# nomic-ai/contrastors

Measured on AMD Instinct MI355X. Metric: query-doc pairs/sec (whole node), nomic-bert-2048 seq128 global-batch 16384, higher is better.
Workload: dtype bf16

## Files before the change

contrastors_amd/csrc/gemm_bf16_v7.hip:

```cpp
#include "cx_common.h"
#include "../../include/contrastors_hip.h"
#include "gemm_params.h"
#include <type_traits>

namespace {

#ifndef CX_V7_NT
#define CX_V7_NT 3
#endif

template <int IMM>
__device__ __forceinline__ void v7_dma_m0(uint32_t base) {
    asm volatile("s_add_u32 m0, %0, %1" ::"s"(base), "n"(IMM) : "memory", "scc");
}
__device__ __forceinline__ void v7_dma_ld(uint32_t off, const bf16_t* base) {
    asm volatile("global_load_lds_dwordx4 %0, %1" ::"v"(off), "s"(base) : "memory");
}
template <int IMM>
__device__ __forceinline__ void v7_dma_full(uint32_t slot_base, uint32_t off, const bf16_t* base) {
    asm volatile("s_add_u32 m0, %0, %1\n\ts_nop 0\n\tglobal_load_lds_dwordx4 %2, %3" ::"s"(slot_base), "n"(IMM), "v"(off), "s"(base)
                 : "memory", "scc");
}
typedef unsigned int v4u7 __attribute__((ext_vector_type(4)));
__device__ __forceinline__ __amdgpu_buffer_rsrc_t rsrc7(const void* base, uint32_t bytes) {
// ... 16 lines not shown
}
template <uint32_t IMM>
__device__ __forceinline__ uint32_t vxor7(uint32_t a) {
    uint32_t r;
    asm volatile("v_xor_b32 %0, %2, %1" : "=v"(r) : "v"(a), "i"(IMM));
    return r;
}

typedef __attribute__((address_space(3))) void* lds_void_ptr7;

constexpr int BM7 = 256, BN7 = 128, BK7 = 64;
constexpr int XW7 = 8192;
constexpr int W0_OFF7 = 32768, SP_OFF7 = 49152, W1_OFF7 = 65536;
constexpr int LDS7 = 81920;

#define V7_MFMA(i, w, x) asm volatile("v_mfma_f32_32x32x16_bf16 %0, %1, %2, %0" : "+a"(acc[(i)]) : "v"(w), "v"(x))
#define V7_MFMA_Z(i, w, x) asm volatile("v_mfma_f32_32x32x16_bf16 %0, %1, %2, 0" : "=a"(acc[(i)]) : "v"(w), "v"(x))

struct XFrags7 {
    bf16x8_t f[2][4];
};
struct WFrags7 {
    bf16x8_t f[4];
};

template <int EPI, int DBG = 0>
__global__ __launch_bounds__(256, 2) __attribute__((amdgpu_waves_per_eu(2, 2))) void gemm_bf16_v7_kernel(GemmParams p) {
    extern __shared__ __attribute__((aligned(16))) char dsm[];
    constexpr bool IS_BWD = EPI == GEMM_EPI_SWIGLU_BWD_AG;
    constexpr bool IS_SWIGLU = EPI == GEMM_EPI_SWIGLU_G;
    static_assert(EPI == GEMM_EPI_NONE || IS_BWD || IS_SWIGLU, "v7 serves the plain / residual, SwiGLU (gate save) and SwiGLU-backward (act, gate) forms");
    const int tid = threadIdx.x;
    const int lane = tid & 63;
    const int wave = __builtin_amdgcn_readfirstlane(tid >> 6);
#ifndef CX_PRODUCT
    long long t_begin = 0;
    if (p.trace) t_begin = (long long)__builtin_amdgcn_s_memtime();
#endif
    const int hi_m = lane >> 5, l31_m = lane & 31;
    const int nk = p.K / BK7;
    const int per_xcd = gridDim.x >> 3;
    const int xcd = blockIdx.x & 7, idx = blockIdx.x >> 3;
    const int gn = p.sup_n > 0 ? p.sup_n : 1, gm = 8 / gn;
    const int xi = xcd / gn, xj = xcd - xi * gn;
    const int m_lo = p.tiles_m * xi / gm, m_hi = p.tiles_m * (xi + 1) / gm;
    const int n_lo = p.tiles_n * xj / gn, n_wd = p.tiles_n * (xj + 1) / gn - n_lo;
    const int nloc = (m_hi - m_lo) * n_wd;
    auto tile_of = [&](int round) {
        const int l = round * per_xcd + idx;
        if (l >= nloc) return -1;
        const int q = l / n_wd;
        return ((m_lo + q) << 8) | (n_lo + (l - q * n_wd));
    };

// ... 72 lines not shown
        for (int i = 0; i < slot * p.sup_m; i += 1024) __builtin_amdgcn_s_sleep(16);
    }
    x_setup(cp_tile);
    w_setup(cp_tile);
    v7_dma_full<0>(x_m0, xoff[0], xbase); v7_dma_full<1024>(x_m0, xoff[1], xbase); v7_dma_full<2048>(x_m0, xoff[2], xbase);
    v7_dma_full<3072>(x_m0, xoff[3], xbase); v7_dma_full<4096>(x_m0, xoff[4], xbase); v7_dma_full<5120>(x_m0, xoff[5], xbase);
    v7_dma_full<6144>(x_m0, xoff[6], xbase); v7_dma_full<7168>(x_m0, xoff[7], xbase);
    x_advance();
    v7_dma_full<0>(w_m0, woff[0], wbase); v7_dma_full<4096>(w_m0, woff[1], wbase); v7_dma_full<8192>(w_m0, woff[2], wbase);
    v7_dma_full<12288>(w_m0, woff[3], wbase);
    w_advance();

    const char* xs = dsm + wave * XW7;
    XFrags7 XF;
    WFrags7 W0, W1;
    f32x16_t acc[8];
    auto read_w = [&](WFrags7& f, const char* ws, int ks, int a) {
        if constexpr ((DBG & 4) != 0) return;
        f.f[a] = lds_read_frag(ws, tile64_off(a * 32 + l31_m, ks * 2 + hi_m));
    };
    auto read_x = [&](int b, int ks) {
        if constexpr ((DBG & 32) != 0) return;
        XF.f[b][ks] = lds_read_frag(xs, tile64_off(b * 32 + l31_m, ks * 2 + hi_m));
    };
    if constexpr ((DBG & (4 | 32 | 8)) != 0) {
#pragma unroll
        for (int a = 0; a < 4; ++a) { W0.f[a] = bf16x8_t{}; W1.f[a] = bf16x8_t{}; }
#pragma unroll
        for (int b = 0; b < 2; ++b)
#pragma unroll
            for (int k = 0; k < 4; ++k) XF.f[b][k] = bf16x8_t{};
#pragma unroll
        for (int i = 0; i < 8; ++i) acc[i] = f32x16_t{};
    }
    int ws_slot = 0;
    asm volatile("s_waitcnt vmcnt(0)" ::: "memory");
    __builtin_amdgcn_s_barrier();
#pragma unroll
    for (int a = 0; a < 4; ++a) read_w(W0, dsm + W0_OFF7, 0, a);

#define V7_M0(kind, J)                                                    \
    do {                                                                  \
        if constexpr ((kind) == 1 && (DBG & 1) == 0) v7_dma_m0<(J) * 4096>(w_m0);           \
        if constexpr ((kind) == 2 && (DBG & 1) == 0) v7_dma_m0<(J) * 1024>(x_m0);           \
    } while (0)
#define V7_LD(kind, J)                                                    \
    do {                                                                  \
        if constexpr ((kind) == 1 && (DBG & 1) == 0) v7_dma_ld(woff[(J)], wbase);           \
        if constexpr ((kind) == 2 && (DBG & 1) == 0) v7_dma_ld(xoff[(J)], xbase);           \
    } while (0)
#define V7_SLOT(MMA, i, WC, ks, kind, J, RD)                              \
    do {                                                                  \
        V7_M0(kind, J);                                                   \
        if constexpr ((DBG & 8) == 0) MMA((i), WC.f[(i) & 3], XF.f[(i) >> 2][(ks)]);   \
        V7_LD(kind, J);                                                   \
        RD;                                                               \
        __builtin_amdgcn_sched_barrier(0);                                \
    } while (0)
#define V7_NORD ((void)0)

    auto kt_body = [&](auto first) {
        const char* ws = dsm + (ws_slot ? W1_OFF7 : W0_OFF7);
        const char* nws = dsm + (ws_slot ? W0_OFF7 : W1_OFF7);
        if constexpr ((DBG & 64) == 0) asm volatile("s_waitcnt vmcnt(0)" ::: "memory");
        read_x(0, 0); read_x(1, 0);
        __builtin_amdgcn_sched_barrier(0);
        read_x(0, 1); read_x(1, 1); read_x(0, 2); read_x(1, 2); read_x(0, 3); read_x(1, 3);
        __builtin_amdgcn_sched_barrier(0);
        if constexpr (decltype(first)::value) {
            V7_SLOT(V7_MFMA_Z, 0, W0, 0, 0, 0, read_w(W1, ws, 1, 0));
            V7_SLOT(V7_MFMA_Z, 1, W0, 0, 1, 0, read_w(W1, ws, 1, 1));
            V7_SLOT(V7_MFMA_Z, 2, W0, 0, 1, 1, read_w(W1, ws, 1, 2));
            V7_SLOT(V7_MFMA_Z, 3, W0, 0, 1, 2, read_w(W1, ws, 1, 3));
            V7_SLOT(V7_MFMA_Z, 4, W0, 0, 1, 3, V7_NORD);
            asm volatile("s_waitcnt lgkmcnt(4)" ::: "memory");
            V7_SLOT(V7_MFMA_Z, 5, W0, 0, 2, 0, V7_NORD);
            V7_SLOT(V7_MFMA_Z, 6, W0, 0, 2, 1, V7_NORD);
            V7_SLOT(V7_MFMA_Z, 7, W0, 0, 2, 2, V7_NORD);
        } else {
            V7_SLOT(V7_MFMA, 0, W0, 0, 0, 0, read_w(W1, ws, 1, 0));
            V7_SLOT(V7_MFMA, 1, W0, 0, 1, 0, read_w(W1, ws, 1, 1));
            V7_SLOT(V7_MFMA, 2, W0, 0, 1, 1, read_w(W1, ws, 1, 2));
            V7_SLOT(V7_MFMA, 3, W0, 0, 1, 2, read_w(W1, ws, 1, 3));
            V7_SLOT(V7_MFMA, 4, W0, 0, 1, 3, V7_NORD);
            asm volatile("s_waitcnt lgkmcnt(4)" ::: "memory");
            V7_SLOT(V7_MFMA, 5, W0, 0, 2, 0, V7_NORD);
            V7_SLOT(V7_MFMA, 6, W0, 0, 2, 1, V7_NORD);
            V7_SLOT(V7_MFMA, 7, W0, 0, 2, 2, V7_NORD);
        }
        w_advance();
        V7_SLOT(V7_MFMA, 0, W1, 1, 2, 3, read_w(W0, ws, 2, 0));
        V7_SLOT(V7_MFMA, 1, W1, 1, 2, 4, read_w(W0, ws, 2, 1));
        V7_SLOT(V7_MFMA, 2, W1, 1, 2, 5, read_w(W0, ws, 2, 2));
        V7_SLOT(V7_MFMA, 3, W1, 1, 2, 6, read_w(W0, ws, 2, 3));
        V7_SLOT(V7_MFMA, 4, W1, 1, 2, 7, V7_NORD);
        V7_SLOT(V7_MFMA, 5, W1, 1, 0, 0, V7_NORD);
        V7_SLOT(V7_MFMA, 6, W1, 1, 0, 0, V7_NORD);
        V7_SLOT(V7_MFMA, 7, W1, 1, 0, 0, V7_NORD);
        x_advance();
        V7_SLOT(V7_MFMA, 0, W0, 2, 0, 0, read_w(W1, ws, 3, 0));
        V7_SLOT(V7_MFMA, 1, W0, 2, 0, 0, read_w(W1, ws, 3, 1));
        V7_SLOT(V7_MFMA, 2, W0, 2, 0, 0, read_w(W1, ws, 3, 2));
        V7_SLOT(V7_MFMA, 3, W0, 2, 0, 0, read_w(W1, ws, 3, 3));
        V7_SLOT(V7_MFMA, 4, W0, 2, 0, 0, V7_NORD);
        V7_SLOT(V7_MFMA, 5, W0, 2, 0, 0, V7_NORD);
        V7_SLOT(V7_MFMA, 6, W0, 2, 0, 0, V7_NORD);
        V7_SLOT(V7_MFMA, 7, W0, 2, 0, 0, V7_NORD);
        asm volatile("s_waitcnt lgkmcnt(0)" ::: "memory");
        if constexpr ((DBG & 64) == 0) asm volatile("s_waitcnt vmcnt(8)" ::: "memory");
        if constexpr ((DBG & 2) == 0) __builtin_amdgcn_s_barrier();
        V7_SLOT(V7_MFMA, 0, W1, 3, 0, 0, read_w(W0, nws, 0, 0));
        V7_SLOT(V7_MFMA, 1, W1, 3, 0, 0, read_w(W0, nws, 0, 1));
        V7_SLOT(V7_MFMA, 2, W1, 3, 0, 0, read_w(W0, nws, 0, 2));
        V7_SLOT(V7_MFMA, 3, W1, 3, 0, 0, read_w(W0, nws, 0, 3));
        V7_SLOT(V7_MFMA, 4, W1, 3, 0, 0, V7_NORD);
        V7_SLOT(V7_MFMA, 5, W1, 3, 0, 0, V7_NORD);
        V7_SLOT(V7_MFMA, 6, W1, 3, 0, 0, V7_NORD);
        V7_SLOT(V7_MFMA, 7, W1, 3, 0, 0, V7_NORD);
        ws_slot ^= 1;
    };

#pragma unroll 1
    while (cp_tile >= 0) {
        if (p.dbg & 1) __builtin_amdgcn_s_setprio(1);
        kt_body(std::true_type{});
#pragma unroll 1
        for (int kt = 1; kt < nk; ++kt) kt_body(std::false_type{});

        if (p.dbg & 1) __builtin_amdgcn_s_setprio(0);
        asm volatile("s_nop 7\n\ts_nop 7\n\ts_nop 7" : "+a"(acc[0]), "+a"(acc[1]), "+a"(acc[2]), "+a"(acc[3]), "+a"(acc[4]), "+a"(acc[5]), "+a"(acc[6]), "+a"(acc[7]));
        int le = lane;
        asm volatile("" : "+v"(le));
        const int hi = le >> 5, l31 = le & 31;
        const int tn = cp_tile & 255, tm = cp_tile >> 8;
        const int m0 = tm * BM7 + wave * 64, n0 = tn * BN7;
        const int rows_left = p.M - m0;
        const uint32_t rows_here = rows_left >= 64 ? 64u : (rows_left > 0 ? (uint32_t)rows_left : 0u);
        const uint32_t my = (uint32_t)((ws_slot ? W0_OFF7 : SP_OFF7) + wave * 8192);
        const uint32_t cb = my + (uint32_t)l31 * 256 + ((l31 & 15) << 4) + hi * 8;
        const int lrow = le >> 4, lch = le & 15;
        const uint32_t rb = my + (uint32_t)lrow * 256 + ((lch ^ lrow) << 4);
#define V7_CELL(c) (dsm + vxor7<((c) << 4)>(cb))
#define V7_ROW(i) (dsm + vxor7<(((i) & 3) << 6)>(rb) + 1024 * (i))
        if constexpr ((DBG & 16) != 0) {
        } else if constexpr (EPI == GEMM_EPI_NONE) {
            const bf16_t* resid = reinterpret_cast<const bf16_t*>(p.Out2);
            const __amdgpu_buffer_rsrc_t rs_out = rsrc7(reinterpret_cast<bf16_t*>(p.Out) + (size_t)m0 * p.ldo + n0, rows_here * (uint32_t)p.ldo * 2u);
            const uint32_t vo = ((uint32_t)lrow * (uint32_t)p.ldo + lch * 8) * 2u;
            const uint32_t so = (uint32_t)p.ldo * 8u;
            auto add_res = [&](uint4& v, const uint4& r) {
                v.x = pack_bf16x2(bf16lo_to_f32(v.x) + bf16lo_to_f32(r.x), bf16hi_to_f32(v.x) + bf16hi_to_f32(r.x));
                v.y = pack_bf16x2(bf16lo_to_f32(v.y) + bf16lo_to_f32(r.y), bf16hi_to_f32(v.y) + bf16hi_to_f32(r.y));
                v.z = pack_bf16x2(bf16lo_to_f32(v.z) + bf16lo_to_f32(r.z), bf16hi_to_f32(v.z) + bf16hi_to_f32(r.z));
                v.w = pack_bf16x2(bf16lo_to_f32(v.w) + bf16lo_to_f32(r.w), bf16hi_to_f32(v.w) + bf16hi_to_f32(r.w));
            };
            auto tile_epi = [&](auto with_resid, auto with_bias) {
                constexpr bool RES = decltype(with_resid)::value;
                constexpr bool BIAS = decltype(with_bias)::value;
                const __amdgpu_buffer_rsrc_t rs_bias = rsrc7(BIAS ? p.bias + n0 : nullptr, BIAS ? (uint32_t)BN7 * 4u : 0u);
                const __amdgpu_buffer_rsrc_t rs_res = rsrc7(RES ? resid + (size_t)m0 * p.ldo2 + n0 : nullptr, RES ? rows_here * (uint32_t)p.ldo2 * 2u : 0u);
                const uint32_t vr = ((uint32_t)lrow * (uint32_t)p.ldo2 + lch * 8) * 2u;
                const uint32_t sr = (uint32_t)p.ldo2 * 8u;
                uint4 r0 = {}, r1 = {}, r2 = {}, r3 = {}, r4 = {}, r5 = {}, r6 = {}, r7 = {};
#define V7_RES_ROWS(b_)                                                                                                     \
    r0 = bld7(rs_res, vr, sr * (8 * (b_) + 0)); r1 = bld7(rs_res, vr, sr * (8 * (b_) + 1)); r2 = bld7(rs_res, vr, sr * (8 * (b_) + 2)); \
    r3 = bld7(rs_res, vr, sr * (8 * (b_) + 3)); r4 = bld7(rs_res, vr, sr * (8 * (b_) + 4)); r5 = bld7(rs_res, vr, sr * (8 * (b_) + 5)); \
    r6 = bld7(rs_res, vr, sr * (8 * (b_) + 6)); r7 = bld7(rs_res, vr, sr * (8 * (b_) + 7));
                auto stage_pass = [&](auto bc) {
                    constexpr int b = decltype(bc)::value;
#pragma unroll
                    for (int a = 0; a < 4; ++a) {
                        uint2 pk[4];
                        float4 bq[4] = {};
                        if constexpr (BIAS) {
#pragma unroll
                            for (int q = 0; q < 4; ++q) bq[q] = bldf7(rs_bias, (uint32_t)hi * 16u, (uint32_t)(a * 128 + q * 32));
                        }
#pragma unroll
                        for (int q = 0; q < 4; ++q) {
                            pk[q].x = pack_bf16x2(acc[4 * b + a][4 * q] + bq[q].x, acc[4 * b + a][4 * q + 1] + bq[q].y);
                            pk[q].y = pack_bf16x2(acc[4 * b + a][4 * q + 2] + bq[q].z, acc[4 * b + a][4 * q + 3] + bq[q].w);
                        }
                        if (a == 0) { *reinterpret_cast<uint2*>(V7_CELL(0)) = pk[0]; *reinterpret_cast<uint2*>(V7_CELL(1)) = pk[1]; *reinterpret_cast<uint2*>(V7_CELL(2)) = pk[2]; *reinterpret_cast<uint2*>(V7_CELL(3)) = pk[3]; }
                        if (a == 1) { *reinterpret_cast<uint2*>(V7_CELL(4)) = pk[0]; *reinterpret_cast<uint2*>(V7_CELL(5)) = pk[1]; *reinterpret_cast<uint2*>(V7_CELL(6)) = pk[2]; *reinterpret_cast<uint2*>(V7_CELL(7)) = pk[3]; }
                        if (a == 2) { *reinterpret_cast<uint2*>(V7_CELL(8)) = pk[0]; *reinterpret_cast<uint2*>(V7_CELL(9)) = pk[1]; *reinterpret_cast<uint2*>(V7_CELL(10)) = pk[2]; *reinterpret_cast<uint2*>(V7_CELL(11)) = pk[3]; }
                        if (a == 3) { *reinterpret_cast<uint2*>(V7_CELL(12)) = pk[0]; *reinterpret_cast<uint2*>(V7_CELL(13)) = pk[1]; *reinterpret_cast<uint2*>(V7_CELL(14)) = pk[2]; *reinterpret_cast<uint2*>(V7_CELL(15)) = pk[3]; }
                        __builtin_amdgcn_sched_barrier(0);
                    }
                };
                auto one_pass = [&](auto bc) {
                    constexpr int b = decltype(bc)::value;
                    uint4 v0 = *reinterpret_cast<const uint4*>(V7_ROW(0)), v1 = *reinterpret_cast<const uint4*>(V7_ROW(1)),
                          v2 = *reinterpret_cast<const uint4*>(V7_ROW(2)), v3 = *reinterpret_cast<const uint4*>(V7_ROW(3)),
                          v4 = *reinterpret_cast<const uint4*>(V7_ROW(4)), v5 = *reinterpret_cast<const uint4*>(V7_ROW(5)),
                          v6 = *reinterpret_cast<const uint4*>(V7_ROW(6)), v7 = *reinterpret_cast<const uint4*>(V7_ROW(7));
                    __builtin_amdgcn_sched_barrier(0);
                    if constexpr (RES) {
                        add_res(v0, r0); add_res(v1, r1); add_res(v2, r2); add_res(v3, r3);
                        add_res(v4, r4); add_res(v5, r5); add_res(v6, r6); add_res(v7, r7);
                        __builtin_amdgcn_sched_barrier(0);
                        if constexpr (b == 0) {
                            V7_RES_ROWS(1)
                            __builtin_amdgcn_sched_barrier(0);
// ... 9 lines not shown
                if constexpr (RES) { V7_RES_ROWS(0) }
                __builtin_amdgcn_sched_barrier(0);
                stage_pass(std::integral_constant<int, 0>{});
                one_pass(std::integral_constant<int, 0>{});
                one_pass(std::integral_constant<int, 1>{});
#undef V7_RES_ROWS
            };
            if (p.bias) {
                if (resid) tile_epi(std::true_type{}, std::true_type{});
                else tile_epi(std::false_type{}, std::true_type{});
            } else {
                if (resid) tile_epi(std::true_type{}, std::false_type{});
                else tile_epi(std::false_type{}, std::false_type{});
            }
        } else if constexpr (IS_SWIGLU) {
            const uint32_t ab = my + (uint32_t)l31 * 128 + ((l31 & 7) << 4) + hi * 8;
            const int arow = le >> 3, ach = le & 7;
            const uint32_t arb = my + (uint32_t)arow * 128 + ((ach ^ arow) << 4);
            const int ncol = (n0 >> 1);
            const __amdgpu_buffer_rsrc_t rs_act = rsrc7(reinterpret_cast<bf16_t*>(p.Out2) + (size_t)m0 * p.ldo2 + ncol, rows_here * (uint32_t)p.ldo2 * 2u);
            const uint32_t va = ((uint32_t)arow * (uint32_t)p.ldo2 + ach * 8) * 2u;
            const uint32_t sa8 = (uint32_t)p.ldo2 * 16u;
            auto swiglu_epi = [&](auto save_c) {
                constexpr bool SAVE = decltype(save_c)::value;
                const __amdgpu_buffer_rsrc_t rs_g = rsrc7(SAVE ? reinterpret_cast<bf16_t*>(p.Out) + (size_t)m0 * p.ldo + ncol : nullptr, SAVE ? rows_here * (uint32_t)p.ldo * 2u : 0u);
                const uint32_t vg = ((uint32_t)arow * (uint32_t)p.ldo + ach * 8) * 2u;
                const uint32_t sg8 = (uint32_t)p.ldo * 16u;
                auto stage_q = [&](auto bc, auto prc, auto qc) {
                    constexpr int b = decltype(bc)::value, pr = decltype(prc)::value, q = decltype(qc)::value;
                    uint2 py, pg;
                    py.x = pack_bf16x2(acc[4 * b + 2 * pr][4 * q], acc[4 * b + 2 * pr][4 * q + 1]);
                    py.y = pack_bf16x2(acc[4 * b + 2 * pr][4 * q + 2], acc[4 * b + 2 * pr][4 * q + 3]);
                    pg.x = pack_bf16x2(acc[4 * b + 2 * pr + 1][4 * q], acc[4 * b + 2 * pr + 1][4 * q + 1]);
                    pg.y = pack_bf16x2(acc[4 * b + 2 * pr + 1][4 * q + 2], acc[4 * b + 2 * pr + 1][4 * q + 3]);
                    const float yy[4] = {bf16lo_to_f32(py.x), bf16hi_to_f32(py.x), bf16lo_to_f32(py.y), bf16hi_to_f32(py.y)};
                    const float gg[4] = {bf16lo_to_f32(pg.x), bf16hi_to_f32(pg.x), bf16lo_to_f32(pg.y), bf16hi_to_f32(pg.y)};
                    float o[4];
#pragma unroll
                    for (int e = 0; e < 4; ++e) o[e] = gg[e] * yy[e] * __builtin_amdgcn_rcpf(1.f + __expf(-gg[e]));
                    uint2 pa;
                    pa.x = pack_bf16x2(o[0], o[1]);
                    pa.y = pack_bf16x2(o[2], o[3]);
                    const uint32_t ca = vxor7<((pr * 4 + q) << 4)>(ab);
                    *reinterpret_cast<uint2*>(dsm + ca) = pa;
                    if constexpr (SAVE) *reinterpret_cast<uint2*>(dsm + ca + 4096) = pg;
                };
                auto stage_pass = [&](auto bc) {
                    stage_q(bc, std::integral_constant<int, 0>{}, std::integral_constant<int, 0>{}); stage_q(bc, std::integral_constant<int, 0>{}, std::integral_constant<int, 1>{});
                    stage_q(bc, std::integral_constant<int, 0>{}, std::integral_constant<int, 2>{}); stage_q(bc, std::integral_constant<int, 0>{}, std::integral_constant<int, 3>{});
                    __builtin_amdgcn_sched_barrier(0);
                    stage_q(bc, std::integral_constant<int, 1>{}, std::integral_constant<int, 0>{}); stage_q(bc, std::integral_constant<int, 1>{}, std::integral_constant<int, 1>{});
                    stage_q(bc, std::integral_constant<int, 1>{}, std::integral_constant<int, 2>{}); stage_q(bc, std::integral_constant<int, 1>{}, std::integral_constant<int, 3>{});
                    __builtin_amdgcn_sched_barrier(0);
                };
                auto one_pass = [&](auto bc) {
                    constexpr int b = decltype(bc)::value;
                    const char* sa = dsm + arb;
                    const uint4 a0 = *reinterpret_cast<const uint4*>(sa), a1 = *reinterpret_cast<const uint4*>(sa + 1024),
// ... 23 lines not shown
            const __amdgpu_buffer_rsrc_t rs_a = rsrc7(reinterpret_cast<const bf16_t*>(p.Out2) + (size_t)m0 * p.ldo2 + n0, rows_here * (uint32_t)p.ldo2 * 2u);
            const __amdgpu_buffer_rsrc_t rs_g = rsrc7(p.In3 + (size_t)m0 * p.ldo2 + n0, rows_here * (uint32_t)p.ldo2 * 2u);
            const __amdgpu_buffer_rsrc_t rs_d = rsrc7(reinterpret_cast<bf16_t*>(p.Out) + (size_t)m0 * p.ldo + 2 * n0, rows_here * (uint32_t)p.ldo * 2u);
            const int r8 = le >> 3, c8 = le & 7;
            const uint32_t vs = ((uint32_t)r8 * (uint32_t)p.ldo2 + c8 * 8) * 2u;
            const uint32_t ss8 = (uint32_t)p.ldo2 * 16u;
            const uint32_t sb = my + (uint32_t)r8 * 256 + (((((c8 >> 2) << 3) | (c8 & 3)) ^ r8) << 4);
            const uint32_t vd = ((uint32_t)lrow * (uint32_t)p.ldo + lch * 8) * 2u;
            const uint32_t sd4 = (uint32_t)p.ldo * 8u;
            uint4 ta0, ta1, ta2, ta3, tg0, tg1, tg2, tg3;
#define V7_LOAD(b_, ap_)                                                                                                                   \
    ta0 = bld7(rs_a, vs + (ap_) * 128, ss8 * (4 * (b_) + 0)); tg0 = bld7(rs_g, vs + (ap_) * 128, ss8 * (4 * (b_) + 0));                    \
    ta1 = bld7(rs_a, vs + (ap_) * 128, ss8 * (4 * (b_) + 1)); tg1 = bld7(rs_g, vs + (ap_) * 128, ss8 * (4 * (b_) + 1));                    \
    ta2 = bld7(rs_a, vs + (ap_) * 128, ss8 * (4 * (b_) + 2)); tg2 = bld7(rs_g, vs + (ap_) * 128, ss8 * (4 * (b_) + 2));                    \
    ta3 = bld7(rs_a, vs + (ap_) * 128, ss8 * (4 * (b_) + 3)); tg3 = bld7(rs_g, vs + (ap_) * 128, ss8 * (4 * (b_) + 3));
            auto cell_q = [&](auto blkc, auto aac, auto qc) {
                constexpr int blk = decltype(blkc)::value, aa = decltype(aac)::value, q = decltype(qc)::value;
                const uint32_t oy = vxor7<((aa * 8 + q) << 4)>(cb);
                const uint32_t og = vxor7<64>(oy);
                char* py = dsm + oy;
                char* pg = dsm + og;
                const uint2 yy = *reinterpret_cast<const uint2*>(py);
                const uint2 gg = *reinterpret_cast<const uint2*>(pg);
                const float y[4] = {bf16lo_to_f32(yy.x), bf16hi_to_f32(yy.x), bf16lo_to_f32(yy.y), bf16hi_to_f32(yy.y)};
                const float g[4] = {bf16lo_to_f32(gg.x), bf16hi_to_f32(gg.x), bf16lo_to_f32(gg.y), bf16hi_to_f32(gg.y)};
                const float d[4] = {acc[blk + aa][4 * q], acc[blk + aa][4 * q + 1], acc[blk + aa][4 * q + 2], acc[blk + aa][4 * q + 3]};
                float dy[4], dg[4];
#pragma unroll
                for (int h = 0; h < 2; ++h) {
                    cx_f2 y2, g2;
                    swiglu_bwd_from_act2(cx_f2{d[2 * h], d[2 * h + 1]}, cx_f2{y[2 * h], y[2 * h + 1]}, cx_f2{g[2 * h], g[2 * h + 1]}, y2, g2);
                    dy[2 * h] = y2.x; dy[2 * h + 1] = y2.y;
                    dg[2 * h] = g2.x; dg[2 * h + 1] = g2.y;
                }
                uint2 o;
                o.x = pack_bf16x2(dy[0], dy[1]); o.y = pack_bf16x2(dy[2], dy[3]);
                *reinterpret_cast<uint2*>(py) = o;
                o.x = pack_bf16x2(dg[0], dg[1]); o.y = pack_bf16x2(dg[2], dg[3]);
                *reinterpret_cast<uint2*>(pg) = o;
            };
            auto one_pass = [&](auto pc) {
                constexpr int ps = decltype(pc)::value;
                constexpr int b = ps >> 1, ap = ps & 1;
                {
                    const uint32_t s0 = sb, s1 = vxor7<128>(sb);
                    *reinterpret_cast<uint4*>(dsm + s0) = ta0; *reinterpret_cast<uint4*>(dsm + (s0 ^ 64)) = tg0;
                    *reinterpret_cast<uint4*>(dsm + s1 + 2048) = ta1; *reinterpret_cast<uint4*>(dsm + (s1 ^ 64) + 2048) = tg1;
                    *reinterpret_cast<uint4*>(dsm + s0 + 4096) = ta2; *reinterpret_cast<uint4*>(dsm + (s0 ^ 64) + 4096) = tg2;
                    *reinterpret_cast<uint4*>(dsm + s1 + 6144) = ta3; *reinterpret_cast<uint4*>(dsm + (s1 ^ 64) + 6144) = tg3;
                }
                __builtin_amdgcn_sched_barrier(0);
                if constexpr (ps < 3) { V7_LOAD((ps + 1) >> 1, (ps + 1) & 1) }
                __builtin_amdgcn_sched_barrier(0);
                constexpr int blk = 4 * b + 2 * ap;
                cell_q(std::integral_constant<int, blk>{}, std::integral_constant<int, 0>{}, std::integral_constant<int, 0>{});
                cell_q(std::integral_constant<int, blk>{}, std::integral_constant<int, 0>{}, std::integral_constant<int, 1>{});
                __builtin_amdgcn_sched_barrier(0);
                cell_q(std::integral_constant<int, blk>{}, std::integral_constant<int, 0>{}, std::integral_constant<int, 2>{});
                cell_q(std::integral_constant<int, blk>{}, std::integral_constant<int, 0>{}, std::integral_constant<int, 3>{});
                __builtin_amdgcn_sched_barrier(0);
                cell_q(std::integral_constant<int, blk>{}, std::integral_constant<int, 1>{}, std::integral_constant<int, 0>{});
                cell_q(std::integral_constant<int, blk>{}, std::integral_constant<int, 1>{}, std::integral_constant<int, 1>{});
                __builtin_amdgcn_sched_barrier(0);
                cell_q(std::integral_constant<int, blk>{}, std::integral_constant<int, 1>{}, std::integral_constant<int, 2>{});
                cell_q(std::integral_constant<int, blk>{}, std::integral_constant<int, 1>{}, std::integral_constant<int, 3>{});
                __builtin_amdgcn_sched_barrier(0);
                auto store_half = [&](auto hc) {
                    constexpr int h = decltype(hc)::value;
                    const uint4 v0 = *reinterpret_cast<const uint4*>(V7_ROW(4 * h + 0)), v1 = *reinterpret_cast<const uint4*>(V7_ROW(4 * h + 1)),
                                v2 = *reinterpret_cast<const uint4*>(V7_ROW(4 * h + 2)), v3 = *reinterpret_cast<const uint4*>(V7_ROW(4 * h + 3));
                    bst7(rs_d, vd + ap * 256, sd4 * (8 * b + 4 * h + 0), v0); bst7(rs_d, vd + ap * 256, sd4 * (8 * b + 4 * h + 1), v1);
                    bst7(rs_d, vd + ap * 256, sd4 * (8 * b + 4 * h + 2), v2); bst7(rs_d, vd + ap * 256, sd4 * (8 * b + 4 * h + 3), v3);
                    __builtin_amdgcn_sched_barrier(0);
                };
                store_half(std::integral_constant<int, 0>{});
                store_half(std::integral_constant<int, 1>{});
            };
            V7_LOAD(0, 0)
            __builtin_amdgcn_sched_barrier(0);
            one_pass(std::integral_constant<int, 0>{});
            one_pass(std::integral_constant<int, 1>{});
// ... 6 lines not shown
        cp_tile = tile_of(++cp_round);
        asm volatile("" : "=v"(W0.f[0]), "=v"(W0.f[1]), "=v"(W0.f[2]), "=v"(W0.f[3]));
        asm volatile("" : "=v"(xoff[0]), "=v"(xoff[1]), "=v"(xoff[2]), "=v"(xoff[3]), "=v"(xoff[4]), "=v"(xoff[5]), "=v"(xoff[6]), "=v"(xoff[7]));
        asm volatile("" : "=v"(woff[0]), "=v"(woff[1]), "=v"(woff[2]), "=v"(woff[3]));
        {
            x_clamped = w_clamped = true;
            const int tx = tile_of(lx_round), tw = tile_of(lw_round);
            x_setup(tx >= 0 ? tx : first_tile);
            xbase += lx_kt * BK7;
            w_setup(tw >= 0 ? tw : first_tile);
            wbase += lw_kt * BK7;
        }
        if (cp_tile >= 0) {
            const char* nws = dsm + (ws_slot ? W1_OFF7 : W0_OFF7);
#pragma unroll
            for (int a = 0; a < 4; ++a) read_w(W0, nws, 0, a);
        }
        asm volatile("s_waitcnt lgkmcnt(0)" ::: "memory");
        __builtin_amdgcn_s_barrier();
    }
#undef V7_SLOT
#undef V7_M0
#undef V7_LD
#undef V7_NORD
    asm volatile("s_waitcnt vmcnt(0)" ::: "memory");
#ifndef CX_PRODUCT
    if (p.trace && tid == 0) {
        unsigned hw, xcc;
        asm volatile("s_getreg_b32 %0, hwreg(HW_REG_HW_ID)" : "=s"(hw));
        asm volatile("s_getreg_b32 %0, hwreg(HW_REG_XCC_ID)" : "=s"(xcc));
        p.trace[4 * blockIdx.x] = t_begin;
        p.trace[4 * blockIdx.x + 1] = (long long)__builtin_amdgcn_s_memtime();
        p.trace[4 * blockIdx.x + 2] = hw;
        p.trace[4 * blockIdx.x + 3] = xcc;
    }
#endif
}

template <int EPI, int DBG = 0>
// ... 97 lines not shown
```

Measured before the change: 4343.

## Switch v7 GEMM from 32x32x16 to 16x16x32 MFMA with spread DMA schedule

Replaces the 32x32x16 bf16 MFMA tiling with 16x16x32 instructions, giving 32 four-register accumulators per wave in place of 8 sixteen-register ones. Fragment reads, the LDS epilogue staging swizzles, and the SwiGLU/backward epilogues are remapped to the new lane layout. The main loop is regenerated as 64 slots per k-tile from a static slot table, with DMA issue and LDS fragment reads spread at configurable intervals. A separate last-iteration body adds a hazard-padded tail MFMA. The aim is better MFMA issue interleaving with memory ops; the risk is more instructions per k-step and a different LDS bank-conflict profile.

Result: no change. 4344, median of 6 (+0.0%).

```diff
diff --git a/contrastors_amd/csrc/gemm_bf16_v7.hip b/contrastors_amd/csrc/gemm_bf16_v7.hip
--- a/contrastors_amd/csrc/gemm_bf16_v7.hip
+++ b/contrastors_amd/csrc/gemm_bf16_v7.hip
@@ -54,15 +54,31 @@
 constexpr int W0_OFF7 = 32768, SP_OFF7 = 49152, W1_OFF7 = 65536;
 constexpr int LDS7 = 81920;
 
-#define V7_MFMA(i, w, x) asm volatile("v_mfma_f32_32x32x16_bf16 %0, %1, %2, %0" : "+a"(acc[(i)]) : "v"(w), "v"(x))
-#define V7_MFMA_Z(i, w, x) asm volatile("v_mfma_f32_32x32x16_bf16 %0, %1, %2, 0" : "=a"(acc[(i)]) : "v"(w), "v"(x))
+#include "gemm_v7_acc.inc"
 
 struct XFrags7 {
-    bf16x8_t f[2][4];
+    bf16x8_t f[4][2];
 };
 struct WFrags7 {
     bf16x8_t f[4];
 };
+
+template <int I0, int I1, class F>
+CX_DEVICE void v7_static_for(F&& f) {
+    if constexpr (I0 < I1) {
+        f(std::integral_constant<int, I0>{});
+        v7_static_for<I0 + 1, I1>(f);
+    }
+}
+
+#ifndef CX_V7_DMA_SPREAD
+#define CX_V7_DMA_SPREAD 4
+#endif
+#ifndef CX_V7_RD_SPREAD
+#define CX_V7_RD_SPREAD 2
+#endif
+static_assert(17 + 7 * CX_V7_DMA_SPREAD < 48 && 3 * CX_V7_DMA_SPREAD < 16, "the W DMAs fit the first quarter, the X DMAs end in front of the barrier");
+static_assert(7 * CX_V7_RD_SPREAD < 16, "the 8 fragment reads of the first quarter fit it");
 
 template <int EPI, int DBG = 0>
 __global__ __launch_bounds__(256, 2) __attribute__((amdgpu_waves_per_eu(2, 2))) void gemm_bf16_v7_kernel(GemmParams p) {
@@ -77,7 +93,7 @@
     long long t_begin = 0;
     if (p.trace) t_begin = (long long)__builtin_amdgcn_s_memtime();
 #endif
-    const int hi_m = lane >> 5, l31_m = lane & 31;
+    const int g4_m = lane >> 4, l15_m = lane & 15;
     const int nk = p.K / BK7;
     const int per_xcd = gridDim.x >> 3;
     const int xcd = blockIdx.x & 7, idx = blockIdx.x >> 3;
@@ -180,30 +196,30 @@
     const char* xs = dsm + wave * XW7;
     XFrags7 XF;
     WFrags7 W0, W1;
-    f32x16_t acc[8];
-    auto read_w = [&](WFrags7& f, const char* ws, int ks, int a) {
+    f32x4_t acc[V7_NACC];
+    auto read_w = [&](WFrags7& f, const char* ws, int kk, int h, int j) {
         if constexpr ((DBG & 4) != 0) return;
-        f.f[a] = lds_read_frag(ws, tile64_off(a * 32 + l31_m, ks * 2 + hi_m));
+        f.f[j] = lds_read_frag(ws, tile64_off((4 * h + j) * 16 + l15_m, kk * 4 + g4_m));
     };
-    auto read_x = [&](int b, int ks) {
+    auto read_x = [&](int mb, int kk) {
         if constexpr ((DBG & 32) != 0) return;
-        XF.f[b][ks] = lds_read_frag(xs, tile64_off(b * 32 + l31_m, ks * 2 + hi_m));
+        XF.f[mb][kk] = lds_read_frag(xs, tile64_off(mb * 16 + l15_m, kk * 4 + g4_m));
     };
     if constexpr ((DBG & (4 | 32 | 8)) != 0) {
 #pragma unroll
-        for (int a = 0; a < 4; ++a) { W0.f[a] = bf16x8_t{}; W1.f[a] = bf16x8_t{}; }
-#pragma unroll
-        for (int b = 0; b < 2; ++b)
-#pragma unroll
-            for (int k = 0; k < 4; ++k) XF.f[b][k] = bf16x8_t{};
-#pragma unroll
-        for (int i = 0; i < 8; ++i) acc[i] = f32x16_t{};
+        for (int j = 0; j < 4; ++j) { W0.f[j] = bf16x8_t{}; W1.f[j] = bf16x8_t{}; }
+#pragma unroll
+        for (int mb = 0; mb < 4; ++mb)
+#pragma unroll
+            for (int k = 0; k < 2; ++k) XF.f[mb][k] = bf16x8_t{};
+#pragma unroll
+        for (int i = 0; i < V7_NACC; ++i) acc[i] = f32x4_t{};
     }
     int ws_slot = 0;
     asm volatile("s_waitcnt vmcnt(0)" ::: "memory");
     __builtin_amdgcn_s_barrier();
 #pragma unroll
-    for (int a = 0; a < 4; ++a) read_w(W0, dsm + W0_OFF7, 0, a);
+    for (int j = 0; j < 4; ++j) read_w(W0, dsm + W0_OFF7, 0, 0, j);
 
 #define V7_M0(kind, J)                                                    \
     do {                                                                  \
@@ -215,98 +231,101 @@
         if constexpr ((kind) == 1 && (DBG & 1) == 0) v7_dma_ld(woff[(J)], wbase);           \
         if constexpr ((kind) == 2 && (DBG & 1) == 0) v7_dma_ld(xoff[(J)], xbase);           \
     } while (0)
-#define V7_SLOT(MMA, i, WC, ks, kind, J, RD)                              \
-    do {                                                                  \
-        V7_M0(kind, J);                                                   \
-        if constexpr ((DBG & 8) == 0) MMA((i), WC.f[(i) & 3], XF.f[(i) >> 2][(ks)]);   \
-        V7_LD(kind, J);                                                   \
-        RD;                                                               \
-        __builtin_amdgcn_sched_barrier(0);                                \
+#define V7_QUARTER(MMA, Q, WC, RD)                                                                         \
+    do {                                                                                                   \
+        v7_static_for<16 * (Q), 16 * (Q) + 16>([&](auto sc_) __attribute__((always_inline)) {              \
+            constexpr int S_ = decltype(sc_)::value, I_ = S_ & 15;                                         \
+            constexpr int DS_ = CX_V7_DMA_SPREAD, RS_ = CX_V7_RD_SPREAD;                                   \
+            constexpr bool DW_ = S_ >= 1 && (S_ - 1) % DS_ == 0 && (S_ - 1) / DS_ < 4;                     \
+            constexpr bool DX_ = S_ >= 17 && (S_ - 17) % DS_ == 0 && (S_ - 17) / DS_ < 8;                  \
+            constexpr int KIND_ = DW_ ? 1 : DX_ ? 2 : 0;                                                   \
+            constexpr int J_ = DW_ ? (S_ - 1) / DS_ : DX_ ? (S_ - 17) / DS_ : 0;                           \
+            if constexpr (I_ % RS_ == 0 && I_ / RS_ < 8) RD(std::integral_constant<int, I_ / RS_>{});      \
+            V7_M0(KIND_, J_);                                                                              \
+            if constexpr ((DBG & 8) != 0) {                                                                \
+            } else if constexpr (S_ == 63 && LAST_) {                                                      \
+                V7_MFMA_TAIL(V7_SLOT[S_][0], WC.f[V7_SLOT[S_][1]], XF.f[V7_SLOT[S_][2]][V7_SLOT[S_][3]]);  \
+            } else {                                                                                       \
+                MMA(V7_SLOT[S_][0], WC.f[V7_SLOT[S_][1]], XF.f[V7_SLOT[S_][2]][V7_SLOT[S_][3]]);           \
+            }                                                                                              \
+            V7_LD(KIND_, J_);                                                                              \
+            __builtin_amdgcn_sched_barrier(0);                                                             \
+            if constexpr (S_ == 15) asm volatile("s_waitcnt lgkmcnt(4)" ::: "memory");                     \
+        });                                                                                                \
     } while (0)
-#define V7_NORD ((void)0)
-
-    auto kt_body = [&](auto first) {
+
+#define V7_MFMA_TAIL(i, w, x) \
+    asm volatile("v_mfma_f32_16x16x32_bf16 %0, %1, %2, %0\n\ts_nop 7\n\ts_nop 7\n\ts_nop 7" : "+a"(acc[(i)]) : "v"(w), "v"(x))
+    auto kt_body = [&](auto first, auto last) {
+        constexpr bool LAST_ = decltype(last)::value;
         const char* ws = dsm + (ws_slot ? W1_OFF7 : W0_OFF7);
         const char* nws = dsm + (ws_slot ? W0_OFF7 : W1_OFF7);
         if constexpr ((DBG & 64) == 0) asm volatile("s_waitcnt vmcnt(0)" ::: "memory");
-        read_x(0, 0); read_x(1, 0);
+        read_x(0, 0); read_x(1, 0); read_x(2, 0); read_x(3, 0);
         __builtin_amdgcn_sched_barrier(0);
-        read_x(0, 1); read_x(1, 1); read_x(0, 2); read_x(1, 2); read_x(0, 3); read_x(1, 3);
-        __builtin_amdgcn_sched_barrier(0);
+        auto rd_q0 = [&](auto rc) __attribute__((always_inline)) {
+            constexpr int r = decltype(rc)::value;
+            if constexpr (r < 4) read_x(r, 1);
+            else read_w(W1, ws, 0, 1, r - 4);
+        };
+        auto rd_q1 = [&](auto rc) __attribute__((always_inline)) {
+            constexpr int r = decltype(rc)::value;
+            if constexpr (r < 4) read_w(W0, ws, 1, 0, r);
+        };
+        auto rd_q2 = [&](auto rc) __attribute__((always_inline)) {
+            constexpr int r = decltype(rc)::value;
+            if constexpr (r < 4) read_w(W1, ws, 1, 1, r);
+        };
+        auto rd_q3 = [&](auto rc) __attribute__((always_inline)) {
+            constexpr int r = decltype(rc)::value;
+            if constexpr (r < 4) read_w(W0, nws, 0, 0, r);
+        };
         if constexpr (decltype(first)::value) {
-            V7_SLOT(V7_MFMA_Z, 0, W0, 0, 0, 0, read_w(W1, ws, 1, 0));
-            V7_SLOT(V7_MFMA_Z, 1, W0, 0, 1, 0, read_w(W1, ws, 1, 1));
-            V7_SLOT(V7_MFMA_Z, 2, W0, 0, 1, 1, read_w(W1, ws, 1, 2));
-            V7_SLOT(V7_MFMA_Z, 3, W0, 0, 1, 2, read_w(W1, ws, 1, 3));
-            V7_SLOT(V7_MFMA_Z, 4, W0, 0, 1, 3, V7_NORD);
-            asm volatile("s_waitcnt lgkmcnt(4)" ::: "memory");
-            V7_SLOT(V7_MFMA_Z, 5, W0, 0, 2, 0, V7_NORD);
-            V7_SLOT(V7_MFMA_Z, 6, W0, 0, 2, 1, V7_NORD);
-            V7_SLOT(V7_MFMA_Z, 7, W0, 0, 2, 2, V7_NORD);
+            V7_QUARTER(V7_MFMA_Z, 0, W0, rd_q0);
         } else {
-            V7_SLOT(V7_MFMA, 0, W0, 0, 0, 0, read_w(W1, ws, 1, 0));
-            V7_SLOT(V7_MFMA, 1, W0, 0, 1, 0, read_w(W1, ws, 1, 1));
-            V7_SLOT(V7_MFMA, 2, W0, 0, 1, 1, read_w(W1, ws, 1, 2));
-            V7_SLOT(V7_MFMA, 3, W0, 0, 1, 2, read_w(W1, ws, 1, 3));
-            V7_SLOT(V7_MFMA, 4, W0, 0, 1, 3, V7_NORD);
-            asm volatile("s_waitcnt lgkmcnt(4)" ::: "memory");
-            V7_SLOT(V7_MFMA, 5, W0, 0, 2, 0, V7_NORD);
-            V7_SLOT(V7_MFMA, 6, W0, 0, 2, 1, V7_NORD);
-            V7_SLOT(V7_MFMA, 7, W0, 0, 2, 2, V7_NORD);
+            V7_QUARTER(V7_MFMA, 0, W0, rd_q0);
         }
         w_advance();
-        V7_SLOT(V7_MFMA, 0, W1, 1, 2, 3, read_w(W0, ws, 2, 0));
-        V7_SLOT(V7_MFMA, 1, W1, 1, 2, 4, read_w(W0, ws, 2, 1));
-        V7_SLOT(V7_MFMA, 2, W1, 1, 2, 5, read_w(W0, ws, 2, 2));
-        V7_SLOT(V7_MFMA, 3, W1, 1, 2, 6, read_w(W0, ws, 2, 3));
-        V7_SLOT(V7_MFMA, 4, W1, 1, 2, 7, V7_NORD);
-        V7_SLOT(V7_MFMA, 5, W1, 1, 0, 0, V7_NORD);
-        V7_SLOT(V7_MFMA, 6, W1, 1, 0, 0, V7_NORD);
-        V7_SLOT(V7_MFMA, 7, W1, 1, 0, 0, V7_NORD);
+        if constexpr (decltype(first)::value) {
+            V7_QUARTER(V7_MFMA_Z, 1, W1, rd_q1);
+        } else {
+            V7_QUARTER(V7_MFMA, 1, W1, rd_q1);
+        }
+        V7_QUARTER(V7_MFMA, 2, W0, rd_q2);
         x_advance();
-        V7_SLOT(V7_MFMA, 0, W0, 2, 0, 0, read_w(W1, ws, 3, 0));
-        V7_SLOT(V7_MFMA, 1, W0, 2, 0, 0, read_w(W1, ws, 3, 1));
-        V7_SLOT(V7_MFMA, 2, W0, 2, 0, 0, read_w(W1, ws, 3, 2));
-        V7_SLOT(V7_MFMA, 3, W0, 2, 0, 0, read_w(W1, ws, 3, 3));
-        V7_SLOT(V7_MFMA, 4, W0, 2, 0, 0, V7_NORD);
-        V7_SLOT(V7_MFMA, 5, W0, 2, 0, 0, V7_NORD);
-        V7_SLOT(V7_MFMA, 6, W0, 2, 0, 0, V7_NORD);
-        V7_SLOT(V7_MFMA, 7, W0, 2, 0, 0, V7_NORD);
         asm volatile("s_waitcnt lgkmcnt(0)" ::: "memory");
         if constexpr ((DBG & 64) == 0) asm volatile("s_waitcnt vmcnt(8)" ::: "memory");
         if constexpr ((DBG & 2) == 0) __builtin_amdgcn_s_barrier();
-        V7_SLOT(V7_MFMA, 0, W1, 3, 0, 0, read_w(W0, nws, 0, 0));
-        V7_SLOT(V7_MFMA, 1, W1, 3, 0, 0, read_w(W0, nws, 0, 1));
-        V7_SLOT(V7_MFMA, 2, W1, 3, 0, 0, read_w(W0, nws, 0, 2));
-        V7_SLOT(V7_MFMA, 3, W1, 3, 0, 0, read_w(W0, nws, 0, 3));
-        V7_SLOT(V7_MFMA, 4, W1, 3, 0, 0, V7_NORD);
-        V7_SLOT(V7_MFMA, 5, W1, 3, 0, 0, V7_NORD);
-        V7_SLOT(V7_MFMA, 6, W1, 3, 0, 0, V7_NORD);
-        V7_SLOT(V7_MFMA, 7, W1, 3, 0, 0, V7_NORD);
+        V7_QUARTER(V7_MFMA, 3, W1, rd_q3);
         ws_slot ^= 1;
     };
 
 #pragma unroll 1
     while (cp_tile >= 0) {
         if (p.dbg & 1) __builtin_amdgcn_s_setprio(1);
-        kt_body(std::true_type{});
+        kt_body(std::true_type{}, std::false_type{});
 #pragma unroll 1
-        for (int kt = 1; kt < nk; ++kt) kt_body(std::false_type{});
+        for (int kt = 2; kt < nk; ++kt) kt_body(std::false_type{}, std::false_type{});
+        kt_body(std::false_type{}, std::true_type{});
 
         if (p.dbg & 1) __builtin_amdgcn_s_setprio(0);
-        asm volatile("s_nop 7\n\ts_nop 7\n\ts_nop 7" : "+a"(acc[0]), "+a"(acc[1]), "+a"(acc[2]), "+a"(acc[3]), "+a"(acc[4]), "+a"(acc[5]), "+a"(acc[6]), "+a"(acc[7]));
+        asm volatile("s_nop 7\n\ts_nop 7\n\ts_nop 7" : "+a"(acc[0]), "+a"(acc[1]), "+a"(acc[2]), "+a"(acc[3]), "+a"(acc[4]), "+a"(acc[5]), "+a"(acc[6]), "+a"(acc[7]),
+                     "+a"(acc[8]), "+a"(acc[9]), "+a"(acc[10]), "+a"(acc[11]), "+a"(acc[12]), "+a"(acc[13]), "+a"(acc[14]));
+        asm volatile("" : "+a"(acc[15]), "+a"(acc[16]), "+a"(acc[17]), "+a"(acc[18]), "+a"(acc[19]), "+a"(acc[20]), "+a"(acc[21]), "+a"(acc[22]),
+                     "+a"(acc[23]), "+a"(acc[24]), "+a"(acc[25]), "+a"(acc[26]), "+a"(acc[27]), "+a"(acc[28]), "+a"(acc[29]));
+        asm volatile("" : "+a"(acc[30]), "+a"(acc[31]));
         int le = lane;
         asm volatile("" : "+v"(le));
-        const int hi = le >> 5, l31 = le & 31;
+        const int g4 = le >> 4, l15 = le & 15;
         const int tn = cp_tile & 255, tm = cp_tile >> 8;
         const int m0 = tm * BM7 + wave * 64, n0 = tn * BN7;
         const int rows_left = p.M - m0;
         const uint32_t rows_here = rows_left >= 64 ? 64u : (rows_left > 0 ? (uint32_t)rows_left : 0u);
         const uint32_t my = (uint32_t)((ws_slot ? W0_OFF7 : SP_OFF7) + wave * 8192);
-        const uint32_t cb = my + (uint32_t)l31 * 256 + ((l31 & 15) << 4) + hi * 8;
+        const uint32_t cb = my + (uint32_t)l15 * 256 + ((l15 ^ (g4 >> 1)) << 4) + (g4 & 1) * 8;
         const int lrow = le >> 4, lch = le & 15;
         const uint32_t rb = my + (uint32_t)lrow * 256 + ((lch ^ lrow) << 4);
-#define V7_CELL(c) (dsm + vxor7<((c) << 4)>(cb))
+#define V7_CELL(nb, mh) (dsm + vxor7<((nb) << 5)>(cb) + 4096 * (mh))
 #define V7_ROW(i) (dsm + vxor7<(((i) & 3) << 6)>(rb) + 1024 * (i))
         if constexpr ((DBG & 16) != 0) {
         } else if constexpr (EPI == GEMM_EPI_NONE) {
@@ -334,25 +353,20 @@
     r6 = bld7(rs_res, vr, sr * (8 * (b_) + 6)); r7 = bld7(rs_res, vr, sr * (8 * (b_) + 7));
                 auto stage_pass = [&](auto bc) {
                     constexpr int b = decltype(bc)::value;
-#pragma unroll
-                    for (int a = 0; a < 4; ++a) {
-                        uint2 pk[4];
-                        float4 bq[4] = {};
-                        if constexpr (BIAS) {
-#pragma unroll
-                            for (int q = 0; q < 4; ++q) bq[q] = bldf7(rs_bias, (uint32_t)hi * 16u, (uint32_t)(a * 128 + q * 32));
+                    v7_static_for<0, 8>([&](auto nbc) __attribute__((always_inline)) {
+                        constexpr int nb = decltype(nbc)::value;
+                        float4 bq = {};
+                        if constexpr (BIAS) bq = bldf7(rs_bias, (uint32_t)g4 * 16u, (uint32_t)(nb * 64));
+#pragma unroll
+                        for (int mh = 0; mh < 2; ++mh) {
+                            const f32x4_t c = acc[v7_blk(2 * b + mh, nb)];
+                            uint2 pk;
+                            pk.x = pack_bf16x2(c[0] + bq.x, c[1] + bq.y);
+                            pk.y = pack_bf16x2(c[2] + bq.z, c[3] + bq.w);
+                            *reinterpret_cast<uint2*>(V7_CELL(nb, mh)) = pk;
                         }
-#pragma unroll
-                        for (int q = 0; q < 4; ++q) {
-                            pk[q].x = pack_bf16x2(acc[4 * b + a][4 * q] + bq[q].x, acc[4 * b + a][4 * q + 1] + bq[q].y);
-                            pk[q].y = pack_bf16x2(acc[4 * b + a][4 * q + 2] + bq[q].z, acc[4 * b + a][4 * q + 3] + bq[q].w);
-                        }
-                        if (a == 0) { *reinterpret_cast<uint2*>(V7_CELL(0)) = pk[0]; *reinterpret_cast<uint2*>(V7_CELL(1)) = pk[1]; *reinterpret_cast<uint2*>(V7_CELL(2)) = pk[2]; *reinterpret_cast<uint2*>(V7_CELL(3)) = pk[3]; }
-                        if (a == 1) { *reinterpret_cast<uint2*>(V7_CELL(4)) = pk[0]; *reinterpret_cast<uint2*>(V7_CELL(5)) = pk[1]; *reinterpret_cast<uint2*>(V7_CELL(6)) = pk[2]; *reinterpret_cast<uint2*>(V7_CELL(7)) = pk[3]; }
-                        if (a == 2) { *reinterpret_cast<uint2*>(V7_CELL(8)) = pk[0]; *reinterpret_cast<uint2*>(V7_CELL(9)) = pk[1]; *reinterpret_cast<uint2*>(V7_CELL(10)) = pk[2]; *reinterpret_cast<uint2*>(V7_CELL(11)) = pk[3]; }
-                        if (a == 3) { *reinterpret_cast<uint2*>(V7_CELL(12)) = pk[0]; *reinterpret_cast<uint2*>(V7_CELL(13)) = pk[1]; *reinterpret_cast<uint2*>(V7_CELL(14)) = pk[2]; *reinterpret_cast<uint2*>(V7_CELL(15)) = pk[3]; }
-                        __builtin_amdgcn_sched_barrier(0);
-                    }
+                        if constexpr ((nb & 1) == 1) __builtin_amdgcn_sched_barrier(0);
+                    });
                 };
                 auto one_pass = [&](auto bc) {
                     constexpr int b = decltype(bc)::value;
@@ -392,7 +406,7 @@
                 else tile_epi(std::false_type{}, std::false_type{});
             }
         } else if constexpr (IS_SWIGLU) {
-            const uint32_t ab = my + (uint32_t)l31 * 128 + ((l31 & 7) << 4) + hi * 8;
+            const uint32_t ab = my + (uint32_t)l15 * 128 + (((l15 & 7) ^ (g4 >> 1)) << 4) + (g4 & 1) * 8;
             const int arow = le >> 3, ach = le & 7;
             const uint32_t arb = my + (uint32_t)arow * 128 + ((ach ^ arow) << 4);
             const int ncol = (n0 >> 1);
@@ -406,11 +420,13 @@
                 const uint32_t sg8 = (uint32_t)p.ldo * 16u;
                 auto stage_q = [&](auto bc, auto prc, auto qc) {
                     constexpr int b = decltype(bc)::value, pr = decltype(prc)::value, q = decltype(qc)::value;
+                    constexpr int mh = q >> 1, nbl = q & 1;
+                    const f32x4_t cy = acc[v7_blk(2 * b + mh, 4 * pr + nbl)], cg = acc[v7_blk(2 * b + mh, 4 * pr + 2 + nbl)];
                     uint2 py, pg;
-                    py.x = pack_bf16x2(acc[4 * b + 2 * pr][4 * q], acc[4 * b + 2 * pr][4 * q + 1]);
-                    py.y = pack_bf16x2(acc[4 * b + 2 * pr][4 * q + 2], acc[4 * b + 2 * pr][4 * q + 3]);
-                    pg.x = pack_bf16x2(acc[4 * b + 2 * pr + 1][4 * q], acc[4 * b + 2 * pr + 1][4 * q + 1]);
-                    pg.y = pack_bf16x2(acc[4 * b + 2 * pr + 1][4 * q + 2], acc[4 * b + 2 * pr + 1][4 * q + 3]);
+                    py.x = pack_bf16x2(cy[0], cy[1]);
+                    py.y = pack_bf16x2(cy[2], cy[3]);
+                    pg.x = pack_bf16x2(cg[0], cg[1]);
+                    pg.y = pack_bf16x2(cg[2], cg[3]);
                     const float yy[4] = {bf16lo_to_f32(py.x), bf16hi_to_f32(py.x), bf16lo_to_f32(py.y), bf16hi_to_f32(py.y)};
                     const float gg[4] = {bf16lo_to_f32(pg.x), bf16hi_to_f32(pg.x), bf16lo_to_f32(pg.y), bf16hi_to_f32(pg.y)};
                     float o[4];
@@ -419,7 +435,7 @@
                     uint2 pa;
                     pa.x = pack_bf16x2(o[0], o[1]);
                     pa.y = pack_bf16x2(o[2], o[3]);
-                    const uint32_t ca = vxor7<((pr * 4 + q) << 4)>(ab);
+                    const uint32_t ca = vxor7<((pr * 4 + nbl * 2) << 4)>(ab) + 2048 * mh;
                     *reinterpret_cast<uint2*>(dsm + ca) = pa;
                     if constexpr (SAVE) *reinterpret_cast<uint2*>(dsm + ca + 4096) = pg;
                 };
@@ -473,17 +489,18 @@
     ta1 = bld7(rs_a, vs + (ap_) * 128, ss8 * (4 * (b_) + 1)); tg1 = bld7(rs_g, vs + (ap_) * 128, ss8 * (4 * (b_) + 1));                    \
     ta2 = bld7(rs_a, vs + (ap_) * 128, ss8 * (4 * (b_) + 2)); tg2 = bld7(rs_g, vs + (ap_) * 128, ss8 * (4 * (b_) + 2));                    \
     ta3 = bld7(rs_a, vs + (ap_) * 128, ss8 * (4 * (b_) + 3)); tg3 = bld7(rs_g, vs + (ap_) * 128, ss8 * (4 * (b_) + 3));
-            auto cell_q = [&](auto blkc, auto aac, auto qc) {
-                constexpr int blk = decltype(blkc)::value, aa = decltype(aac)::value, q = decltype(qc)::value;
-                const uint32_t oy = vxor7<((aa * 8 + q) << 4)>(cb);
+            auto cell_ptr = [&](auto aac, auto nblc, auto mhc, char*& py, char*& pg) __attribute__((always_inline)) {
+                constexpr int aa = decltype(aac)::value, nbl = decltype(nblc)::value, mh = decltype(mhc)::value;
+                const uint32_t oy = vxor7<((aa * 8 + nbl * 2) << 4)>(cb);
                 const uint32_t og = vxor7<64>(oy);
-                char* py = dsm + oy;
-                char* pg = dsm + og;
-                const uint2 yy = *reinterpret_cast<const uint2*>(py);
-                const uint2 gg = *reinterpret_cast<const uint2*>(pg);
+                py = dsm + oy + 4096 * mh;
+                pg = dsm + og + 4096 * mh;
+            };
+            auto cell_q = [&](auto blkc, char* py, char* pg, const uint2 yy, const uint2 gg) __attribute__((always_inline)) {
+                constexpr int blk = decltype(blkc)::value;
                 const float y[4] = {bf16lo_to_f32(yy.x), bf16hi_to_f32(yy.x), bf16lo_to_f32(yy.y), bf16hi_to_f32(yy.y)};
                 const float g[4] = {bf16lo_to_f32(gg.x), bf16hi_to_f32(gg.x), bf16lo_to_f32(gg.y), bf16hi_to_f32(gg.y)};
-                const float d[4] = {acc[blk + aa][4 * q], acc[blk + aa][4 * q + 1], acc[blk + aa][4 * q + 2], acc[blk + aa][4 * q + 3]};
+                const float d[4] = {acc[blk][0], acc[blk][1], acc[blk][2], acc[blk][3]};
                 float dy[4], dg[4];
 #pragma unroll
                 for (int h = 0; h < 2; ++h) {
@@ -511,19 +528,23 @@
                 __builtin_amdgcn_sched_barrier(0);
                 if constexpr (ps < 3) { V7_LOAD((ps + 1) >> 1, (ps + 1) & 1) }
                 __builtin_amdgcn_sched_barrier(0);
-                constexpr int blk = 4 * b + 2 * ap;
-                cell_q(std::integral_constant<int, blk>{}, std::integral_constant<int, 0>{}, std::integral_constant<int, 0>{});
-                cell_q(std::integral_constant<int, blk>{}, std::integral_constant<int, 0>{}, std::integral_constant<int, 1>{});
-                __builtin_amdgcn_sched_barrier(0);
-                cell_q(std::integral_constant<int, blk>{}, std::integral_constant<int, 0>{}, std::integral_constant<int, 2>{});
-                cell_q(std::integral_constant<int, blk>{}, std::integral_constant<int, 0>{}, std::integral_constant<int, 3>{});
-                __builtin_amdgcn_sched_barrier(0);
-                cell_q(std::integral_constant<int, blk>{}, std::integral_constant<int, 1>{}, std::integral_constant<int, 0>{});
-                cell_q(std::integral_constant<int, blk>{}, std::integral_constant<int, 1>{}, std::integral_constant<int, 1>{});
-                __builtin_amdgcn_sched_barrier(0);
-                cell_q(std::integral_constant<int, blk>{}, std::integral_constant<int, 1>{}, std::integral_constant<int, 2>{});
-                cell_q(std::integral_constant<int, blk>{}, std::integral_constant<int, 1>{}, std::integral_constant<int, 3>{});
-                __builtin_amdgcn_sched_barrier(0);
+                v7_static_for<0, 2>([&](auto mhc) __attribute__((always_inline)) {
+                    constexpr int mh = decltype(mhc)::value;
+                    char *py[4], *pg[4];
+                    uint2 yy[4], gg[4];
+                    v7_static_for<0, 4>([&](auto cc) __attribute__((always_inline)) {
+                        constexpr int c = decltype(cc)::value;
+                        cell_ptr(std::integral_constant<int, (c >> 1)>{}, std::integral_constant<int, (c & 1)>{}, mhc, py[c], pg[c]);
+                        yy[c] = *reinterpret_cast<const uint2*>(py[c]);
+                        gg[c] = *reinterpret_cast<const uint2*>(pg[c]);
+                    });
+                    __builtin_amdgcn_sched_barrier(0);
+                    v7_static_for<0, 4>([&](auto cc) __attribute__((always_inline)) {
+                        constexpr int c = decltype(cc)::value;
+                        cell_q(std::integral_constant<int, v7_blk(2 * b + mh, 4 * ap + c)>{}, py[c], pg[c], yy[c], gg[c]);
+                        if constexpr (c & 1) __builtin_amdgcn_sched_barrier(0);
+                    });
+                });
                 auto store_half = [&](auto hc) {
                     constexpr int h = decltype(hc)::value;
                     const uint4 v0 = *reinterpret_cast<const uint4*>(V7_ROW(4 * h + 0)), v1 = *reinterpret_cast<const uint4*>(V7_ROW(4 * h + 1)),
@@ -560,15 +581,15 @@
         if (cp_tile >= 0) {
             const char* nws = dsm + (ws_slot ? W1_OFF7 : W0_OFF7);
 #pragma unroll
-            for (int a = 0; a < 4; ++a) read_w(W0, nws, 0, a);
+            for (int j = 0; j < 4; ++j) read_w(W0, nws, 0, 0, j);
         }
         asm volatile("s_waitcnt lgkmcnt(0)" ::: "memory");
         __builtin_amdgcn_s_barrier();
     }
-#undef V7_SLOT
+#undef V7_QUARTER
+#undef V7_MFMA_TAIL
 #undef V7_M0
 #undef V7_LD
-#undef V7_NORD
     asm volatile("s_waitcnt vmcnt(0)" ::: "memory");
 #ifndef CX_PRODUCT
     if (p.trace && tid == 0) {
diff --git a/contrastors_amd/csrc/gemm_v7_acc.inc b/contrastors_amd/csrc/gemm_v7_acc.inc
--- /dev/null
+++ b/contrastors_amd/csrc/gemm_v7_acc.inc
@@ -0,0 +1,26 @@
+
+#define V7_MFMA(i, w, x) asm volatile("v_mfma_f32_16x16x32_bf16 %0, %1, %2, %0" : "+a"(acc[(i)]) : "v"(w), "v"(x))
+#define V7_MFMA_Z(i, w, x) asm volatile("v_mfma_f32_16x16x32_bf16 %0, %1, %2, 0" : "=a"(acc[(i)]) : "v"(w), "v"(x))
+
+constexpr int V7_NACC = 32;
+constexpr int v7_blk(int mb, int nb) { return 8 * mb + nb; }
+constexpr int v7_region_blk(int b, int a, int q) { return v7_blk(2 * b + (q >> 1), 2 * a + (q & 1)); }
+
+constexpr unsigned char V7_SLOT[64][4] = {
+    {0, 0, 0, 0}, {1, 1, 0, 0}, {2, 2, 0, 0}, {3, 3, 0, 0},
+    {8, 0, 1, 0}, {9, 1, 1, 0}, {10, 2, 1, 0}, {11, 3, 1, 0},
+    {16, 0, 2, 0}, {17, 1, 2, 0}, {18, 2, 2, 0}, {19, 3, 2, 0},
+    {24, 0, 3, 0}, {25, 1, 3, 0}, {26, 2, 3, 0}, {27, 3, 3, 0},
+    {4, 0, 0, 0}, {5, 1, 0, 0}, {6, 2, 0, 0}, {7, 3, 0, 0},
+    {12, 0, 1, 0}, {13, 1, 1, 0}, {14, 2, 1, 0}, {15, 3, 1, 0},
+    {20, 0, 2, 0}, {21, 1, 2, 0}, {22, 2, 2, 0}, {23, 3, 2, 0},
+    {28, 0, 3, 0}, {29, 1, 3, 0}, {30, 2, 3, 0}, {31, 3, 3, 0},
+    {0, 0, 0, 1}, {1, 1, 0, 1}, {2, 2, 0, 1}, {3, 3, 0, 1},
+    {8, 0, 1, 1}, {9, 1, 1, 1}, {10, 2, 1, 1}, {11, 3, 1, 1},
+    {16, 0, 2, 1}, {17, 1, 2, 1}, {18, 2, 2, 1}, {19, 3, 2, 1},
+    {24, 0, 3, 1}, {25, 1, 3, 1}, {26, 2, 3, 1}, {27, 3, 3, 1},
+    {4, 0, 0, 1}, {5, 1, 0, 1}, {6, 2, 0, 1}, {7, 3, 0, 1},
+    {12, 0, 1, 1}, {13, 1, 1, 1}, {14, 2, 1, 1}, {15, 3, 1, 1},
+    {20, 0, 2, 1}, {21, 1, 2, 1}, {22, 2, 2, 1}, {23, 3, 2, 1},
+    {28, 0, 3, 1}, {29, 1, 3, 1}, {30, 2, 3, 1}, {31, 3, 3, 1},
+};
```
